# sungnyun/dualhyp

Hardware: AMD Instinct MI355X
Metric: corrected utterances/sec (TinyLlama-1.1B, 5+5 hyps, 512->64 tok) (higher is better)
Workload: dtype bf16; 1 GPU; DualHyp inference, TinyLlama-1.1B bf16 + LoRA r16 (q,k,v,proj), batch 32/GPU synthetic 5+5-hyp prompts, 512-token prompt -> 64 generated tokens, greedy; batch_per_gpu=32, parallelism=replicas x1, batches_in_flight_per_gpu=64, schedule=merged, decode_rows_per_launch=2048

## Files before the change

dualhyp_amd/_lib.py:

```python
from __future__ import annotations

import ctypes as C
from pathlib import Path

_HERE = Path(__file__).resolve().parent
import os as _os
LIB_PATH = Path(_os.environ["DUALHYP_HIP_LIB"]) if _os.environ.get("DUALHYP_HIP_LIB") else _HERE / "lib" / "libdualhyp_hip.so"

P = C.c_void_p
I = C.c_int
I64 = C.c_int64
U64 = C.c_uint64
F = C.c_float


class LayerWeights(C.Structure):
    _fields_ = [(n, P) for n in ("norm_1", "norm_2", "attn_w", "attn_lora_a", "attn_lora_b", "proj_w",
                                 "proj_lora_a", "proj_lora_b", "fc_1", "fc_2", "mlp_proj",
                                 "attn_ws", "proj_ws", "fc_1_ws", "fc_2_ws", "mlp_proj_ws")]


class ModelDesc(C.Structure):
    _fields_ = [("n_layer", C.c_int32), ("n_head", C.c_int32), ("n_groups", C.c_int32), ("head_size", C.c_int32),
                ("n_embd", C.c_int32), ("intermediate", C.c_int32), ("vocab", C.c_int32), ("block_size", C.c_int32),
# ... 24 lines not shown
    "dh_set_tuning": (I, [I, I]),
    "dh_debug_gemm_routes": (U64, [I]),
    "dh_last_error": (C.c_char_p, []),
    "dh_device_info": (I, [C.c_char_p, I, C.POINTER(I), C.POINTER(I64)]),
    "dh_embed_bf16": (I, [P, P, P, I, I, I, P]),
    "dh_rmsnorm_bf16": (I, [P, P, P, P, P, I, I, F, P, P]),
    "dh_qkv_rope_cache_bf16": (I, [P, P, P, P, P, P, P, P, P, P, I, I, I, I, I, P]),
    "dh_linear_bf16": (I, [P, P, P, I, I, I, I, P, P, I, P, F, I, I, P, P, P, P]),
    "dh_linear_qkv_rope_cache_bf16": (I, [P, P, I, I, P, I, P, F, P, P, P, P, P, P, P, I, I, I, I, P]),
    "dh_linear_lora_bf16": (I, [P, P, P, I, I, I, P, P, F, I, I, P, P, P]),
    "dh_linear_qkv_lora_rope_cache_bf16": (I, [P, P, I, I, P, P, F, P, P, P, P, P, P, P, I, I, I, I, P, P]),
    "dh_linear_partial_bf16": (I, [P, P, P, P, I, I, I, I, I, P]),
    "dh_linear_chain_bf16": (I, [P, P, P, P, I, I, I, I, I, P]),
    "dh_linear_partial_pairs_bf16": (I, [P, P, P, P, I, I, I, I, I, P]),
    "dh_finish_norm_bf16": (I, [P, I, I, I, I, I, P, F, P, P, P, P, F, P, P]),
    "dh_attn_decode_fused_bf16": (I, [P, I, I, I, I, I, P, F, I, I, P, P, P, P, P, P, P, I, I, I, I, P]),
    "dh_attn_verify_fused_bf16": (I, [P, I, I, I, I, I, I, P, F, I, I, P, P, P, P, P, P, P, I, I, I, I, I, P]),
    "dh_attn_prefill_bf16": (I, [P, P, P, P, P, P, P, P, P, I, I, I, I, I, I, P]),
    "dh_dropout_bf16": (I, [P, P, P, I64, F, C.c_uint64, C.c_uint32, P, P]),
    "dh_swiglu_fwd_bf16": (I, [P, P, P, I64, P]),
    "dh_linear_swiglu_train_bf16": (I, [P, P, P, P, P, P, I, I, I, P]),
    "dh_linear_mul_bf16": (I, [P, P, P, I, I, I, P, P]),
    "dh_swiglu_bwd_bf16": (I, [P, P, P, P, I, I, P]),
    "dh_rmsnorm_bwd_bf16": (I, [P, P, P, P, P, I, I, F, P]),
    "dh_qkv_rope_bwd_bf16": (I, [P, P, P, P, P, P, P, I, I, I, I, P]),
    "dh_tn_accum_f32": (I, [P, I, P, I, P, I, I, I, I, F, I, P, P]),
    "dh_tn_accum_work_bytes": (I64, [I, I, I]),
    "dh_tn_accum_seg_f32": (I, [P, I, P, I, P, I, I, I, I, I, F, I, P, P]),
    "dh_rowdot_f32": (I, [P, P, P, I64, I, P]),
    "dh_transpose_pad_bf16": (I, [P, P, P, P, P, I, I, I, I, P]),
# ... 115 lines not shown
```

dualhyp_amd/csrc/capi.hip:

```cpp
#include "common.h"
#include "tuning.h"
#include <stdarg.h>

static thread_local char g_err[512] = "";

void dh_set_error(const char* fmt, ...) {
    va_list ap;
    va_start(ap, fmt);
    vsnprintf(g_err, sizeof(g_err), fmt, ap);
    va_end(ap);
}

extern "C" const char* dh_last_error(void) { return g_err; }
extern "C" int dh_abi_version(void) { return DH_ABI_VERSION; }

int dh_stop_pack(const char* name, const dh_stop_spec* stop, bool start_ok, dh_stop_args& out) {
    out = dh_stop_args{};
    if (!stop) return 0;
    DH_CHECK(stop->n_seqs >= 0 && stop->n_seqs <= DH_MAX_STOP_SEQS, "%s: %d stop sequences, at most %d are supported", name, stop->n_seqs,
             DH_MAX_STOP_SEQS);
    DH_CHECK(stop->n_seqs == 0 || (stop->seqs && stop->h_seq_len), "%s: %d stop sequences without their ids or their lengths", name,
             stop->n_seqs);
    uint32_t lens = 0;
    for (int i = 0; i < stop->n_seqs; ++i) {
// ... 108 lines not shown
    {22, &g_w4_persist, RANGE, 0, 2, 0},
    {23, &g_prune_last_layer, BOOL, 0, 0, 0},
    {24, &g_w4_fast_epi, ANY, 0, 0, 0},
    {25, &g_w4_persist_qkv, BOOL, 0, 0, 0},
    {26, &g_tn_mfma, BOOL, 0, 0, 0},
    {27, &g_attn_bwd_dq_group, BOOL, 0, 0, 0},
    {28, &g_tail_split, BOOL, 0, 0, 0},
    {29, &g_attn_bwd_dkdv_img, BOOL, 0, 0, 0},
    {30, &g_w4_persist_lora, BOOL, 0, 0, 0},
    {31, &g_skinny_n, BOOL, 0, 0, 0},
    {40, &g_attn_chain, BOOL, 0, 0, 0},
    {41, &g_finish_hoist_rows, RANGE, -1, NO_MAX, 0},
    {42, &g_prefill_wpb, ONE_OF, 0, 2, 4},
    {43, &g_finish_rows_min, RANGE, -1, NO_MAX, 0},
    {44, &g_finish_rpb, RANGE, 0, 64, 0},
};

}

extern "C" int dh_set_tuning(int key, int value) {
    for (const TuningRow& r : TUNING) {
        if (r.key != key) continue;
        if (r.accept == RANGE && (value < r.a || value > r.b)) break;
        if (r.accept == ONE_OF && value != r.a && value != r.b && value != r.c) break;
        *r.knob = r.accept == BOOL ? value != 0 : value;
        return 0;
    }
    dh_set_error("dh_set_tuning: unknown key %d", key);
    return 1;
}
// ... 1 lines not shown
```

dualhyp_amd/csrc/decode_fused.hip:

```cpp
#include "common.h"
#include "tuning.h"

int g_attn_chain = 1;
int g_finish_hoist_rows = -1;
int g_finish_rows_min = -1;
int g_finish_rpb = 0;

#ifdef DH_ATTN_STAMPS
__device__ unsigned long long g_attn_stamps[4096 * 8];
#define ATTN_STAMP(i) do { if (threadIdx.x == 0 && blockIdx.x < 4096) g_attn_stamps[blockIdx.x * 8 + (i)] = __builtin_amdgcn_s_memrealtime(); } while (0)
#define ATTN_DRAIN() __builtin_amdgcn_s_waitcnt(0)
extern "C" int dh_debug_attn_stamps(unsigned long long* out) {
    return hipMemcpyFromSymbol(out, HIP_SYMBOL(g_attn_stamps), sizeof(g_attn_stamps)) == hipSuccess ? 0 : 1;
}
#else
#define ATTN_STAMP(i)
#define ATTN_DRAIN()
#endif

namespace {

constexpr int DCOLS = 16;
constexpr int MAXP = 16;

// ... 999 lines not shown
            const int c0 = (tid + i * 256) * 8;
            if (c0 < d) {
                const uint4 wu = i == 0 ? hwu : *reinterpret_cast<const uint4*>(w_norm + c0);
                const bf16_t* wp = reinterpret_cast<const bf16_t*>(&wu);
                uint4 o;
                bf16_t* op = reinterpret_cast<bf16_t*>(&o);
#pragma unroll
                for (int e = 0; e < 8; ++e) op[e] = f2bf(bf2f(wp[e]) * rbf(v[i][e] * r));
                *reinterpret_cast<uint4*>(xn_out + (size_t)row * d + c0) = o;
            }
        }
    };
    for (int k = 0; k < nrow; k += 2) {
        do_row(pa, pb, k);
        if (k + 1 < nrow) do_row(pb, pa, k + 1);
    }
}

}

extern "C" int dh_attn_decode_fused_bf16(const float* qkv32, int n_part, int pairs, int n_seq, int qkv_dim, int n_ext,
                                         const dh_bf16* lora_b, float lora_scale, int split0, int split1,
                                         const dh_bf16* cos, const dh_bf16* sin, const int32_t* seq_slot,
                                         const int32_t* kv_len, dh_bf16* k_cache, dh_bf16* vT_cache, dh_bf16* y,
                                         int n_head, int n_groups, int hs, int s_max, void* stream) {
    DH_CHECK(qkv32 && cos && sin && seq_slot && kv_len && k_cache && vT_cache && y, "dh_attn_decode_fused_bf16: null argument");
    DH_CHECK(n_groups > 0 && n_head % n_groups == 0 && n_head / n_groups <= DCOLS, "dh_attn_decode_fused_bf16: bad head counts");
    DH_CHECK(hs == 64 || hs == 96 || hs == 128, "dh_attn_decode_fused_bf16: head_size %d unsupported", hs);
    DH_CHECK(s_max % 64 == 0 && n_part >= 1 && n_part <= MAXP, "dh_attn_decode_fused_bf16: bad s_max / n_part");
    DH_CHECK(qkv_dim == (n_head + 2 * n_groups) * hs, "dh_attn_decode_fused_bf16: qkv_dim mismatch");
// ... 137 lines not shown
        else LAUNCH_MAXC(4);
#undef LAUNCH_MAXC
#undef LAUNCH_ROWS
        DH_LAUNCH_CHECK();
        return 0;
    }
    const int hoist_rows = g_finish_hoist_rows >= 0 ? g_finish_hoist_rows : FINISH_HOIST_ROWS;
    const bool hoist = hoist_rows > 0 && rows >= hoist_rows;
    if (d <= 2048) { LAUNCH(1); }
    else if (d <= 4096) { LAUNCH(2); }
    else { LAUNCH(4); }
#undef LAUNCH
    DH_LAUNCH_CHECK();
    return 0;
}
```

dualhyp_amd/csrc/engine.hip:

```cpp
#include <algorithm>
#include <mutex>
#include <vector>

#include "common.h"
#include "gemm.h"

constexpr int MAX_DECODE_ROWS = 2048;
int g_decode_tiled_rows = 0;
int g_short_kps = 8;
int g_fuse_qkv_rope = 1;
int g_prune_last_layer = 1;

struct dh_engine {
    dh_model_desc d;
    std::vector<dh_layer_weights> layers;
    int max_batch = 0, s_max = 0, max_tokens = 0;
    int row_cap = 0;
    int qkv_dim = 0, kv_dim = 0;
    bf16_t *kc = nullptr, *vtc = nullptr;
    bool kv8 = false;
    uint8_t *k8 = nullptr, *v8 = nullptr;
    int8_t *ke = nullptr, *ve = nullptr;
    size_t exp_layer_elems = 0;
    bf16_t *x = nullptr, *xn = nullptr, *qkv = nullptr, *qrot = nullptr, *att = nullptr, *xa = nullptr,
// ... 41 lines not shown
    hipStream_t gstream = nullptr;
    hipEvent_t ev_in = nullptr, ev_out = nullptr, ev_stage = nullptr;
    struct GKey {
        int64_t* tokens; int tok_ld; int32_t *length, *done; int n_seq, top_k; float temp; int64_t eos; uint64_t seed; int rsqrt_vec, tiled_rows;
        const int32_t *limit, *row_seq, *row_slot; int n_all, max_new;
        int spec; const int64_t* drafts; int32_t* counters;
        float* logprobs;
        int top_n; int32_t* top_ids; float* top_lp;
        const uint32_t* mask; int mask_ld;
        int ngram; const int32_t* ngram_start;
        dh_stop_args stop; const int32_t* stop_start; int32_t* stop_fin_tok;
        dh_nucleus_args nuc;
        dh_penalty_args pen; const int32_t* pen_start;
        dh_bias_args bias; const int32_t* bias_start;
        int beam_w; dh_beam_state beam;
        bool operator==(const GKey& k) const {
            return tokens == k.tokens && tok_ld == k.tok_ld && length == k.length && done == k.done && n_seq == k.n_seq &&
                   top_k == k.top_k && temp == k.temp && eos == k.eos && seed == k.seed && rsqrt_vec == k.rsqrt_vec &&
                   tiled_rows == k.tiled_rows && limit == k.limit && row_seq == k.row_seq && row_slot == k.row_slot &&
                   n_all == k.n_all && max_new == k.max_new && spec == k.spec && drafts == k.drafts && counters == k.counters &&
                   logprobs == k.logprobs && top_n == k.top_n && top_ids == k.top_ids && top_lp == k.top_lp && mask == k.mask &&
                   mask_ld == k.mask_ld && ngram == k.ngram && ngram_start == k.ngram_start && stop == k.stop && stop_start == k.stop_start &&
                   stop_fin_tok == k.stop_fin_tok && nuc == k.nuc && dh_penalty_same(pen, k.pen) && pen_start == k.pen_start &&
                   bias == k.bias && bias_start == k.bias_start &&
                   beam_w == k.beam_w &&
                   memcmp(&beam, &k.beam, sizeof(beam)) == 0;
        }
    };
    struct GEntry { GKey key; hipGraphExec_t exec; uint64_t used; };
    std::vector<GEntry> graphs;
    uint64_t graph_clock = 0;
    const int32_t* seq_slot = nullptr;
    bool capturing = false;
    bool phase_decode = false;
    bool decode_tiled = false;
    struct Timing {
        bool on = false;
        std::vector<std::pair<hipEvent_t, hipEvent_t>> ev[4];
    } tm;
};
// ... 467 lines not shown
            np = ks; pairs = 1;
            return dh_linear_partial_bf16(xin, w, wext, e->part32, n_seq, N, ext, K, ks, s);
        };
        int np, pairs;
        const int ext1 = W.attn_lora_a ? 48 : 0;
        if ((rc = partial(e->xn, W.attn_w, W.attn_lora_a, e->qkv_dim, ext1, d, pick_ksplit(d / 32), np, pairs))) return rc;
        if (spec_S > 1) {
            const int p_max = e->s_max < D.block_size ? e->s_max : D.block_size;
            if ((rc = dh_attn_verify_fused_impl(e->part32, np, pairs, n_seq / spec_S, spec_S, e->qkv_dim, ext1, W.attn_lora_b, D.lora_scale,
                                                d, d + e->kv_dim, D.rope_cos, D.rope_sin, m.seq_slot, m.kv, kc, vtc, e->att, H, G, hs,
                                                e->s_max, p_max, s))) return rc;
        } else
        if ((rc = dh_attn_decode_fused_bf16(e->part32, np, pairs, n_seq, e->qkv_dim, ext1, W.attn_lora_b, D.lora_scale, d,
                                            d + e->kv_dim, D.rope_cos, D.rope_sin, m.seq_slot, m.kv, kc, vtc, e->att, H, G,
                                            hs, e->s_max, s))) return rc;
        const int ext2 = W.proj_lora_a ? 16 : 0;
        if ((rc = partial(e->att, W.proj_w, W.proj_lora_a, d, ext2, d, pick_ksplit(d / 32), np, pairs))) return rc;
        if ((rc = dh_finish_norm_bf16(e->part32, np, pairs, n_seq, d, ext2, W.proj_lora_b, D.lora_scale, e->x, W.norm_2, e->x,
                                      e->xn, D.norm_eps, rt, s))) return rc;
        if ((rc = swiglu(e, e->xn, W.fc_1, W.fc_2, e->act, n_seq, I, d, s, false))) return rc;
        if ((rc = partial(e->act, W.mlp_proj, nullptr, d, 0, I, pick_ksplit(I / 32), np, pairs))) return rc;
        const bf16_t* next_norm = l + 1 < D.n_layer ? e->layers[l + 1].norm_1 : D.ln_f;
        if ((rc = dh_finish_norm_bf16(e->part32, np, pairs, n_seq, d, 0, nullptr, 0.f, e->x, next_norm, e->x, e->xn,
                                      D.norm_eps, rt, s))) return rc;
    }
    return 0;
}

int head(dh_engine* e, const bf16_t* xrows, int rows, bf16_t* logits, const uint8_t* tail_flags, hipStream_t s) {
    const dh_model_desc& D = e->d;
    const uint8_t* rt = e->rsqrt_vec > 0 ? tail_flags : nullptr;
    int rc;
    if (e->fp8) {
        if ((rc = dh_rmsnorm_quant_fp8(xrows, D.ln_f, e->xn, e->xq, e->xscale, rows, D.n_embd, D.norm_eps, rt, s))) return rc;
        TimeScope t(e, gemm_class(e), s);
        return dh_linear_fp8_ex(e->xq, e->xscale, reinterpret_cast<const uint8_t*>(D.lm_head), D.lm_head_ws, logits, rows, D.vocab,
                                D.n_embd, DH_EPI_ADAPTER, nullptr, nullptr, D.adapter_scale, D.adapter_bias, nullptr,
                                fp8_kernel(e->phase_decode, rows), s);
    }
// ... 796 lines not shown
```

dualhyp_amd/csrc/gemm.h:

```cpp
#pragma once
#include "common.h"
#include "tuning.h"

struct GemmArgs {
    const bf16_t* x;
    const bf16_t* w;
    const bf16_t* w2;
    bf16_t* y;
    const bf16_t* xa;
    const bf16_t* lora_a;
    const bf16_t* lora_b;
    const bf16_t* vec_a;
    const bf16_t* vec_b;
    const bf16_t* resid;
    int M, N, K;
    int xa_ld, split0, split1;
    float lora_scale;
    int nb_n, nb_m;
    int gm;
    int fast_epi;
    int resid_mul;
    const bf16_t* rope_cos;
    const bf16_t* rope_sin;
    const int32_t* tok_slot;
// ... 41 lines not shown
bool dh_linear_k64_ok(int M, int N, int K, const void* x, const void* w, const void* y, const void* mul);
int dh_linear_k64(const dh_bf16* x, const dh_bf16* w, const dh_bf16* mul, dh_bf16* y, int M, int N, hipStream_t s);
bool dh_linear_256_xa_ok(const GemmArgs& a, int epilogue);

bool dh_linear_mid_ok(const GemmArgs& a, int epilogue);
int dh_linear_mid(const GemmArgs& a, int epilogue, hipStream_t s);

bool dh_linear_dt_ok(const GemmArgs& a, int epilogue, int seg);
int dh_linear_dt(const GemmArgs& a, int epilogue, int seg, hipStream_t s);
bool dh_chain_ok(int M, int n_main, int n_ext, int K, int ksplit);
bool dh_pairs_ok(int M, int n_main, int n_ext, int K, int ksplit);
int dh_pairs_tiled(const bf16_t* x, const bf16_t* w, const bf16_t* w_ext, float* y32, int M, int n_main, int n_ext, int K,
                   int kps, hipStream_t s);
int dh_chain_tiled(const bf16_t* x, const bf16_t* w, const bf16_t* w_ext, float* y32, int M, int n_main, int n_ext, int K,
                   int kps, hipStream_t s);

bool dh_linear_is_big(int M, int N, int epilogue);

int dh_linear_256(GemmArgs a, int epilogue, hipStream_t s);

int dh_linear_lora_impl(const dh_bf16* x, const dh_bf16* w, dh_bf16* y, int M, int N, int K, const dh_bf16* lora_a, const dh_bf16* lora_b,
                        float lora_scale, int split0, int split1, const dh_bf16* resid, dh_bf16* xa_work, int kernel, hipStream_t s);
int dh_linear_impl(const dh_bf16* x, const dh_bf16* w, dh_bf16* y, int M, int N, int K, int epilogue,
                   const dh_bf16* w2, const dh_bf16* xa, int xa_ld, const dh_bf16* lora_b, float lora_scale,
                   int split0, int split1, const dh_bf16* vec_a, const dh_bf16* vec_b, const dh_bf16* resid,
                   int kernel, hipStream_t s);
```

dualhyp_amd/csrc/gemm_dt.hip:

```cpp
#include "common.h"
#include "gemm.h"

int g_dt_stages = 0;
int g_dt_wide = 0;

namespace {

constexpr int TB = 128;
constexpr int BKD = 64;
template <int WN> constexpr int stage_bytes() { return (WN * 64 + TB) * BKD * 2; }

__device__ __forceinline__ int swz7(int row) { return (row >> 1) & 7; }

struct DtArgs {
    const bf16_t* x;
    const bf16_t* w;
    const bf16_t* w2;
    void* y;
    const bf16_t* vec_a;
    const bf16_t* vec_b;
    const bf16_t* resid;
    int M, N, K, n_main, seg;
    int split_kt;
    int wt;
};

template <int MODE, int NSTAGE, int WN, int WI>
__device__ __forceinline__ void gemm_dt_body(const DtArgs& a) {
    static_assert(WI == 4 || (WI == 2 && MODE == 0 && !(WN == 4 && NSTAGE == 3)), "the 32 x 64 wave tile serves MODE 0 on the plain ring");
    constexpr int STAGE = stage_bytes<WN>();
    constexpr int ASZ = WN * 64 * BKD * 2;
    constexpr int NWV = WN * 8 / WI;
    constexpr int NA = WI;
    constexpr int NB = 16 / NWV;
    constexpr int PER = NA + NB;
    extern __shared__ __attribute__((aligned(16))) char smem[];
    const int tid = threadIdx.x, lane = tid & 63;
    const int wave = WI == 2 ? __builtin_amdgcn_readfirstlane(tid >> 6) : tid >> 6;
    const int wn = wave >> 1, wm = wave & 1;
    const int frow = lane & 15, kg = lane >> 4;
    const int m_tiles = (a.M + TB - 1) / TB;
    int tile, ky = 0;
    {
        const int nwg = gridDim.x * gridDim.y, bid = blockIdx.x + gridDim.x * blockIdx.y, xcd = bid & 7, q = nwg >> 3, r = nwg & 7;
        tile = (xcd < r ? xcd * (q + 1) : r * (q + 1) + (xcd - r) * q) + (bid >> 3);
        if (MODE == 4) { ky = tile / (int)gridDim.x; tile -= ky * (int)gridDim.x; }
    }
    const int tm = tile % m_tiles, tn = tile / m_tiles;
    const int m0 = tm * TB;
    const int n0 = MODE == 1 ? tn * (WN * 32) : tn * (WN * 64);
// ... 16 lines not shown
            n = n0 + row;
            n = n < a.N ? n : a.N - 1;
            if ((MODE == 0 || MODE == 4) && n >= a.n_main) { base = a.w2; n -= a.n_main; }
        }
        srcA[j] = base + (size_t)n * a.K + chunk * 8 + (MODE == 4 ? (size_t)ky * a.split_kt * BKD : 0);
    }
#pragma unroll
    for (int j = 0; j < NB; ++j) {
        const int R = wave * NB + j;
        const int row = R * 8 + (lane >> 3);
        const int chunk = (lane & 7) ^ swz7(row);
        int m = m0 + row;
        m = m < a.M ? m : a.M - 1;
        srcB[j] = a.x + (size_t)m * a.K + chunk * 8 + (MODE == 4 ? (size_t)ky * a.split_kt * BKD : 0);
    }
    auto stage = [&](int kt) __attribute__((always_inline)) {
        char* sA = smem + (kt % NSTAGE) * STAGE;
        char* sB = sA + ASZ;
#pragma unroll
        for (int j = 0; j < NA; ++j) glds16(srcA[j] + kt * BKD, sA + (wave * NA + j) * 1024);
#pragma unroll
        for (int j = 0; j < NB; ++j) glds16(srcB[j] + kt * BKD, sB + (wave * NB + j) * 1024);
    };
    auto wait_next = [&](int ahead) __attribute__((always_inline)) {
        if (NSTAGE >= 4 && ahead >= 2) asm volatile("s_waitcnt vmcnt(%0)" ::"n"(2 * PER) : "memory");
        else if (NSTAGE >= 3 && ahead >= 1) asm volatile("s_waitcnt vmcnt(%0)" ::"n"(PER) : "memory");
        else asm volatile("s_waitcnt vmcnt(0)" ::: "memory");
    };

    f32x4 cur[WI][4], tot[WI][4];
#pragma unroll
    for (int i = 0; i < WI; ++i)
#pragma unroll
        for (int j = 0; j < 4; ++j) {
            cur[i][j] = f32x4{0.f, 0.f, 0.f, 0.f};
            tot[i][j] = f32x4{0.f, 0.f, 0.f, 0.f};
        }
    const int sw = swz7(frow);
    const int offA = (wn * (WI * 16) + frow) * 128, offB = (wm * 64 + frow) * 128;
    const int nk = MODE == 4 ? min(a.split_kt, a.K / BKD - ky * a.split_kt) : a.K / BKD;
    const int seg_kt = a.seg / 2;
    f32x4 pairacc[MODE == 0 ? WI : 1][MODE == 0 ? 4 : 1];
    int seg_idx = 0;

    auto fold_segment = [&](bool last) __attribute__((always_inline)) {
        if (MODE == 0) {
            const bool second = seg_idx & 1;
#pragma unroll
            for (int i = 0; i < WI; ++i)
#pragma unroll
                for (int j = 0; j < 4; ++j) {
                    if (second) tot[i][j] += pairacc[i][j] + cur[i][j];
                    else if (last) tot[i][j] += cur[i][j];
                    else pairacc[i][j] = cur[i][j];
                    cur[i][j] = f32x4{0.f, 0.f, 0.f, 0.f};
                }
            ++seg_idx;
        } else {
#pragma unroll
            for (int i = 0; i < WI; ++i)
#pragma unroll
                for (int j = 0; j < 4; ++j) {
                    tot[i][j] += cur[i][j];
                    cur[i][j] = f32x4{0.f, 0.f, 0.f, 0.f};
                }
        }
    };
    int in_seg = 0;
    if constexpr (WN == 4 && NSTAGE == 3) {
    auto stage_w = [&](int kt) __attribute__((always_inline)) {
        char* sA = smem + (kt % NSTAGE) * STAGE;
// ... 52 lines not shown
        if (p < nk) stage(p);
    wait_next((nk < NSTAGE - 1 ? nk : NSTAGE - 1) - 1);
    __builtin_amdgcn_s_barrier();
    for (int kt = 0; kt < nk; ++kt) {
        const bool pre = kt + NSTAGE - 1 < nk;
        const char* sA = smem + (kt % NSTAGE) * STAGE;
        const char* sB = sA + ASZ;
        if (pre) stage(kt + NSTAGE - 1);
#pragma unroll
        for (int ks = 0; ks < 2; ++ks) {
            const int co = ((ks * 4 + kg) ^ sw) << 4;
            if constexpr (WI == 2) {
                bf16x8 fa[2];
#pragma unroll
                for (int i = 0; i < 2; ++i) fa[i] = *reinterpret_cast<const bf16x8*>(sA + offA + i * 2048 + co);
#pragma unroll
                for (int j = 0; j < 4; ++j) {
                    const bf16x8 fb = *reinterpret_cast<const bf16x8*>(sB + offB + j * 2048 + co);
#pragma unroll
                    for (int i = 0; i < 2; ++i) cur[i][j] = __builtin_amdgcn_mfma_f32_16x16x32_bf16(fa[i], fb, cur[i][j], 0, 0, 0);
                }
            } else {
            bf16x8 fa[4], fb[4];
#pragma unroll
            for (int i = 0; i < 4; ++i) {
                fa[i] = *reinterpret_cast<const bf16x8*>(sA + offA + i * 2048 + co);
                fb[i] = *reinterpret_cast<const bf16x8*>(sB + offB + i * 2048 + co);
            }
#pragma unroll
            for (int i = 0; i < 4; ++i)
// ... 2 lines not shown
                    cur[i][j] = __builtin_amdgcn_mfma_f32_16x16x32_bf16(fa[i], fb[j], cur[i][j], 0, 0, 0);
            }
        }
        if (++in_seg == seg_kt || kt + 1 == nk) {
            in_seg = 0;
            fold_segment(kt + 1 == nk);
        }
        {
            const int issued = (kt + NSTAGE - 1 < nk ? kt + NSTAGE - 1 : nk - 1);
            wait_next(issued - (kt + 1));
        }
        __builtin_amdgcn_s_barrier();
    }
    }

#pragma unroll
    for (int j = 0; j < 4; ++j) {
        const int m = m0 + wm * 64 + j * 16 + frow;
        if (m >= a.M) continue;
        if constexpr (MODE == 1) {
#pragma unroll
            for (int i = 0; i < 2; ++i) {
                const int n = n0 + wn * 32 + i * 16 + kg * 4;
                if (n >= a.N) continue;
                float o[4];
#pragma unroll
                for (int r = 0; r < 4; ++r) {
                    const float gt = rbf(tot[i][j][r]), up = rbf(tot[i + 2][j][r]);
                    o[r] = rbf(silu_fast(gt)) * up;
                }
// ... 23 lines not shown
#pragma unroll
                    for (int r = 0; r < 4; ++r) o[r] = bf2f(rp[r]) + o[r];
                }
                *reinterpret_cast<uint2*>((bf16_t*)a.y + (size_t)m * a.N + n) = make_uint2(pack2bf(o[0], o[1]), pack2bf(o[2], o[3]));
            }
        }
    }
}

template <int MODE, int NSTAGE, int WN = 2>
__global__ __launch_bounds__(WN * 128) void gemm_dt_kernel(DtArgs a) { gemm_dt_body<MODE, NSTAGE, WN, 4>(a); }

template <int NSTAGE>
__global__ __launch_bounds__(512, NSTAGE == 2 ? 4 : 2) void gemm_dt_chain_kernel(DtArgs a) { gemm_dt_body<0, NSTAGE, 2, 2>(a); }

template <int NSTAGE>
int launch_chain_n(const DtArgs& a, int blocks, hipStream_t s) {
    constexpr int lds = NSTAGE * stage_bytes<2>();
    DH_MAX_LDS_ONCE((gemm_dt_chain_kernel<NSTAGE>), lds);
    dh_gemm_route(DH_ROUTE_CHAIN_TILED);
    hipLaunchKernelGGL((gemm_dt_chain_kernel<NSTAGE>), dim3(blocks), dim3(512), lds, s, a);
    DH_LAUNCH_CHECK();
    return 0;
}

template <int MODE, int NSTAGE, int WN = 2>
int launch_dt_n(const DtArgs& a, int blocks, hipStream_t s, int ny = 1) {
    constexpr int lds = NSTAGE * stage_bytes<WN>();
    DH_MAX_LDS_ONCE((gemm_dt_kernel<MODE, NSTAGE, WN>), lds);
    dh_gemm_route(MODE == 0 ? DH_ROUTE_CHAIN_TILED : MODE == 4 ? DH_ROUTE_PAIRS_TILED : DH_ROUTE_DT_FUSED);
// ... 12 lines not shown
    const int stages = g_dt_stages ? g_dt_stages : (blocks > 256 ? 2 : 4);
    return stages == 2 ? launch_dt_n<MODE, 2>(a, blocks, s) : launch_dt_n<MODE, 4>(a, blocks, s);
}

}

int g_dt_min_rows = 129;
int g_chain_min_rows = 1536;

int dh_chain_tiled(const bf16_t* x, const bf16_t* w, const bf16_t* w_ext, float* y32, int M, int n_main, int n_ext, int K,
                   int kps, hipStream_t s) {
    DtArgs a{x, w, w_ext ? w_ext : w, y32, nullptr, nullptr, nullptr, M, n_main + n_ext, K, n_main, kps, 0, 0};
    const int blocks = cdiv(M, TB) * cdiv(a.N, TB);
    const int stages = g_dt_stages ? g_dt_stages : (blocks > 256 ? 2 : 4);
    return stages == 2 ? launch_chain_n<2>(a, blocks, s) : launch_chain_n<4>(a, blocks, s);
}

int g_pairs_wn = 0;
int g_pairs_wt = 0;
int dh_pairs_tiled(const bf16_t* x, const bf16_t* w, const bf16_t* w_ext, float* y32, int M, int n_main, int n_ext, int K,
                   int kps, hipStream_t s) {
    const int N = n_main + n_ext, nslices = cdiv(K / 32, kps), ny = (nslices + 1) / 2;
    DtArgs a{x, w, w_ext ? w_ext : w, y32, nullptr, nullptr, nullptr, M, N, K, n_main, kps, kps, g_pairs_wt};
    const int m_tiles = cdiv(M, TB);
    const int wide_blocks = m_tiles * cdiv(N, 256) * ny;
    const bool wide = g_pairs_wn ? g_pairs_wn == 4 : wide_blocks >= 160;
    if (wide) return launch_dt_n<4, 3, 4>(a, m_tiles * cdiv(N, 256), s, ny);
    const int blocks = m_tiles * cdiv(N, TB);
    return blocks * ny > 256 ? launch_dt_n<4, 2>(a, blocks, s, ny) : launch_dt_n<4, 4>(a, blocks, s, ny);
}
// ... 17 lines not shown
```

dualhyp_amd/csrc/gemm_skinny.hip:

```cpp
#include "common.h"
#include "gemm.h"

int g_skinny_variant = 1;
int g_swiglu2 = 1;
int g_rows_ng = 0;
int g_rows_ct = 0;

namespace {

constexpr int ROWS = 16;
constexpr int NW = 8;
constexpr int CH = 8;

template <int EPI, bool RESID>
__global__ __launch_bounds__(512, 2) void gemm_skinny_kernel(GemmArgs a) {
    __shared__ __attribute__((aligned(16))) float part[NW][32][ROWS];
    __shared__ __attribute__((aligned(16))) float part2[EPI == DH_EPI_SWIGLU ? NW : 1][32][ROWS];
    const int tid = threadIdx.x, lane = tid & 63, wave = tid >> 6;
    const int n0 = blockIdx.x * ROWS;
    const int lrow = lane & 15, kg = lane >> 4;
    constexpr bool SW = EPI == DH_EPI_SWIGLU;
    constexpr int CHK = SW ? CH / 2 : CH;
    const int kw = wave, kstride = NW;
    int n = n0 + lrow;
// ... 571 lines not shown
             n_ext % ROWS == 0, "dh_linear_partial_pairs_bf16: unsupported shape N=%d+%d K=%d ksplit=%d (K %% 64 == 0, whole K-slices of 8 or 16 k-steps)",
             n_main, n_ext, K, ksplit);
    return dh_pairs_tiled(x, w, w_ext, y32, M, n_main, n_ext, K, kps, (hipStream_t)stream);
}

extern "C" int dh_linear_chain_bf16(const dh_bf16* x, const dh_bf16* w, const dh_bf16* w_ext, float* y32, int M, int n_main,
                                    int n_ext, int K, int ksplit, void* stream) {
    DH_CHECK(x && w && y32 && M >= 1 && ksplit >= 1 && (n_ext == 0 || w_ext), "dh_linear_chain_bf16: bad argument");
    DH_CHECK(dh_chain_ok(M, n_main, n_ext, K, ksplit),
             "dh_linear_chain_bf16: unsupported shape M=%d N=%d+%d K=%d ksplit=%d (needs >= %d rows, K %% 64 == 0, K-slices of 8 or 16 k-steps)",
             M, n_main, n_ext, K, ksplit, g_chain_min_rows);
    const int kps = (K / 32 + ksplit - 1) / ksplit;
    return dh_chain_tiled(x, w, w_ext, y32, M, n_main, n_ext, K, kps, (hipStream_t)stream);
}

int g_skinny_n = 1;
bool dh_linear_skinny_n_ok(int M, int N, int K, const void* x, const void* w, const void* y) {
    return g_skinny_n && N >= 16 && N <= 64 && N % 16 == 0 && M >= 512 && K >= 64 && K % 64 == 0 && (size_t)M * K * 2 < (1ull << 32) &&
           (((uintptr_t)x | (uintptr_t)w) & 15) == 0 && ((uintptr_t)y & 7) == 0;
}
int dh_linear_skinny_n(const dh_bf16* x, const dh_bf16* w, dh_bf16* y, int M, int N, int K, hipStream_t s) {
    const dim3 grid(cdiv(M, 64)), block(256);
    const int nt = N / 16, lds = 4 * (64 * 128 + nt * 16 * 128);
    dh_gemm_route(DH_ROUTE_SKINNY_N);
    switch (nt) {
        case 1: hipLaunchKernelGGL((gemm_skinny_n_kernel<1>), grid, block, lds, s, x, w, y, M, K, N); break;
        case 2: hipLaunchKernelGGL((gemm_skinny_n_kernel<2>), grid, block, lds, s, x, w, y, M, K, N); break;
        case 3: hipLaunchKernelGGL((gemm_skinny_n_kernel<3>), grid, block, lds, s, x, w, y, M, K, N); break;
        default: hipLaunchKernelGGL((gemm_skinny_n_kernel<4>), grid, block, lds, s, x, w, y, M, K, N); break;
    }
// ... 35 lines not shown
```

dualhyp_amd/csrc/tuning.h:

```cpp
#pragma once

extern int g_gemm128_stages, g_gemm_variant, g_tail_split, g_linear_phase;
extern int g_gemm_gm, g_w4_persist, g_w4_fast_epi, g_w4_persist_qkv, g_w4_persist_lora;
extern int g_mid, g_mid_wlds;
extern int g_dt_stages, g_dt_wide, g_dt_min_rows, g_chain_min_rows, g_pairs_wn, g_pairs_wt;
extern int g_pairs_min_rows, g_skinny_n;
__attribute__((visibility("hidden"))) extern int g_skinny_variant, g_swiglu2, g_rows_ct, g_rows_ng;
extern int g_fp8_tile, g_fp8_gm;
extern int g_decode_tiled_rows, g_short_kps, g_fuse_qkv_rope, g_prune_last_layer;
extern int g_attn_bwd_dkdv_img, g_attn_bwd_dq_group;
extern int g_tn_mfma;
extern int g_attn_chain, g_finish_hoist_rows, g_finish_rows_min, g_finish_rpb;
extern int g_prefill_wpb;
```

dualhyp_amd/ops.py:

```python
from __future__ import annotations

import os
from typing import Sequence, Optional, Tuple

import torch

from . import _lib
from ._lib import check

EPI_PLAIN, EPI_LORA, EPI_SWIGLU, EPI_ADAPTER = 0, 1, 2, 3


def _p(t: Optional[torch.Tensor]):
    return None if t is None else t.data_ptr()


def _stream() -> int:
    return torch.cuda.current_stream().cuda_stream


def _dev(t: torch.Tensor, dtype=torch.bfloat16, name="tensor") -> torch.Tensor:
    if not t.is_cuda:
        raise _lib.DualHypHipError(f"{name} must live on the GPU: the HIP path has no CPU fallback")
    if t.dtype != dtype:
# ... 692 lines not shown
    return y


def finish_norm(h32: torch.Tensor, d: int, x_resid: torch.Tensor, w_norm: torch.Tensor, eps: float,
                lora_b: Optional[torch.Tensor] = None, lora_scale: float = 1.0,
                row_tail: Optional[torch.Tensor] = None, pairs: bool = True) -> Tuple[torch.Tensor, torch.Tensor]:
    k = _Keep()
    n_part, rows, ld = h32.shape
    x_resid = _dev(x_resid, name="x_resid")
    x_out, xn_out = torch.empty_like(x_resid), torch.empty_like(x_resid)
    check(_lib.load().dh_finish_norm_bf16(_p(h32), n_part, int(pairs), rows, d, ld - d, _p(lora_b), float(lora_scale), _p(x_resid),
                                          k(w_norm), _p(x_out), _p(xn_out), float(eps), _p(row_tail), _stream()))
    return x_out, xn_out


def attn_decode_fused(qkv32: torch.Tensor, qkv_dim: int, lora_b: Optional[torch.Tensor], lora_scale: float,
                      splits: Tuple[int, int], cos: torch.Tensor, sin: torch.Tensor, seq_slot: torch.Tensor,
                      kv_len: torch.Tensor, k_cache: torch.Tensor, vT_cache: torch.Tensor, n_head: int,
                      pairs: bool = True) -> torch.Tensor:
    k = _Keep()
    n_part, n_seq, ld = qkv32.shape
    n_groups, s_max, hs = k_cache.size(1), k_cache.size(2), k_cache.size(3)
    y = torch.empty((n_seq, n_head * hs), dtype=torch.bfloat16, device=qkv32.device)
    i32 = torch.int32
    check(_lib.load().dh_attn_decode_fused_bf16(_p(qkv32), n_part, int(pairs), n_seq, qkv_dim, ld - qkv_dim, _p(lora_b),
                                                float(lora_scale), splits[0], splits[1], k(cos), k(sin),
                                                k(seq_slot, i32), k(kv_len, i32), _p(k_cache), _p(vT_cache),
                                                _p(y), n_head, n_groups, hs, s_max, _stream()))
    return y

# ... 156 lines not shown
```

include/dualhyp_hip.h:

```cpp
#ifndef DUALHYP_HIP_H
#define DUALHYP_HIP_H

#include <stdint.h>

#ifdef __cplusplus
extern "C" {
#endif

typedef uint16_t dh_bf16;

#define DH_ABI_VERSION 6

int dh_abi_version(void);
int dh_set_tuning(int key, int value);
uint64_t dh_debug_gemm_routes(int reset);
const char* dh_last_error(void);
int dh_device_info(char* h_buf, int h_buf_len, int* h_num_cu, int64_t* h_hbm_bytes);


int dh_embed_bf16(const int64_t* ids, const dh_bf16* wte, dh_bf16* out, int n_tok, int d,
                  int vocab, void* stream);

int dh_rmsnorm_bf16(const dh_bf16* x, const dh_bf16* resid, const dh_bf16* w, dh_bf16* out,
                    dh_bf16* sum_out, int rows, int d, float eps, const uint8_t* row_tail,
// ... 29 lines not shown
                                       const int32_t* tok_slot, const int32_t* tok_pos, dh_bf16* q_out, dh_bf16* k_cache,
                                       dh_bf16* vT_cache, int n_head, int n_groups, int hs, int s_max, dh_bf16* xa_work,
                                       void* stream);

int dh_linear_partial_bf16(const dh_bf16* x, const dh_bf16* w, const dh_bf16* w_ext, float* y32,
                           int M, int n_main, int n_ext, int K, int ksplit, void* stream);
int dh_linear_partial_pairs_bf16(const dh_bf16* x, const dh_bf16* w, const dh_bf16* w_ext, float* y32, int M,
                                 int n_main, int n_ext, int K, int ksplit, void* stream);
int dh_linear_chain_bf16(const dh_bf16* x, const dh_bf16* w, const dh_bf16* w_ext, float* y32, int M,
                         int n_main, int n_ext, int K, int ksplit, void* stream);

int dh_finish_norm_bf16(const float* h32, int n_part, int pairs, int rows, int d, int n_ext,
                        const dh_bf16* lora_b, float lora_scale, const dh_bf16* x_resid,
                        const dh_bf16* w_norm, dh_bf16* x_out, dh_bf16* xn_out, float eps,
                        const uint8_t* row_tail, void* stream);


int dh_attn_prefill_bf16(const dh_bf16* q, const dh_bf16* k_cache, const dh_bf16* vT_cache,
                         const int32_t* seq_slot, const int32_t* q_start, const int32_t* q_len,
                         const int32_t* kv_pos0, dh_bf16* y, float* lse, int n_seq, int max_q_len,
                         int n_head, int n_groups, int hs, int s_max, void* stream);

int64_t dh_attn_decode_work_bytes(int n_seq, int n_head, int hs, int s_max);
int dh_attn_decode_bf16(const dh_bf16* q, const dh_bf16* k_cache, const dh_bf16* vT_cache,
                        const int32_t* seq_slot, const int32_t* kv_len, dh_bf16* y, void* work,
                        int n_seq, int n_head, int n_groups, int hs, int s_max, void* stream);

int dh_attn_decode_fused_bf16(const float* qkv32, int n_part, int pairs, int n_seq, int qkv_dim, int n_ext,
                              const dh_bf16* lora_b, float lora_scale, int split0, int split1,
                              const dh_bf16* cos, const dh_bf16* sin, const int32_t* seq_slot,
// ... 347 lines not shown
```

Before: 855.5 utterances/s.

## Fuse residual add and LoRA epilogue into chain GEMM, then separate RMSNorm

In decode, the out-projection and MLP down-projection no longer write fp32 partial sums and reduce them in a finish-norm kernel when the chain shape allows it. A new finishing mode of the tiled chain GEMM computes the LoRA x·A product alongside the main MFMA loop and adds LoRA B plus the residual in its epilogue, writing bf16 x in place. A lightweight row-wise RMSNorm kernel then produces xn. This removes the fp32 partial-buffer traffic, at the cost of an extra norm launch and a heavier GEMM epilogue that adds LDS and register pressure.

```diff
diff --git a/dualhyp_amd/_lib.py b/dualhyp_amd/_lib.py
--- a/dualhyp_amd/_lib.py
+++ b/dualhyp_amd/_lib.py
@@ -62,6 +62,8 @@
     "dh_linear_chain_bf16": (I, [P, P, P, P, I, I, I, I, I, P]),
     "dh_linear_partial_pairs_bf16": (I, [P, P, P, P, I, I, I, I, I, P]),
     "dh_finish_norm_bf16": (I, [P, I, I, I, I, I, P, F, P, P, P, P, F, P, P]),
+    "dh_linear_chain_finish_bf16": (I, [P, P, P, P, F, P, I, I, I, I, P]),
+    "dh_norm_finished_bf16": (I, [P, P, P, I, I, F, P, P]),
     "dh_attn_decode_fused_bf16": (I, [P, I, I, I, I, I, P, F, I, I, P, P, P, P, P, P, P, I, I, I, I, P]),
     "dh_attn_verify_fused_bf16": (I, [P, I, I, I, I, I, I, P, F, I, I, P, P, P, P, P, P, P, I, I, I, I, I, P]),
     "dh_attn_prefill_bf16": (I, [P, P, P, P, P, P, P, P, P, I, I, I, I, I, I, P]),
diff --git a/dualhyp_amd/csrc/capi.hip b/dualhyp_amd/csrc/capi.hip
--- a/dualhyp_amd/csrc/capi.hip
+++ b/dualhyp_amd/csrc/capi.hip
@@ -146,6 +146,7 @@
     {42, &g_prefill_wpb, ONE_OF, 0, 2, 4},
     {43, &g_finish_rows_min, RANGE, -1, NO_MAX, 0},
     {44, &g_finish_rpb, RANGE, 0, 64, 0},
+    {45, &g_chain_finish, BOOL, 0, 0, 0},
 };
 
 }
diff --git a/dualhyp_amd/csrc/decode_fused.hip b/dualhyp_amd/csrc/decode_fused.hip
--- a/dualhyp_amd/csrc/decode_fused.hip
+++ b/dualhyp_amd/csrc/decode_fused.hip
@@ -1037,6 +1037,70 @@
     for (int k = 0; k < nrow; k += 2) {
         do_row(pa, pb, k);
         if (k + 1 < nrow) do_row(pb, pa, k + 1);
+    }
+}
+
+template <int MAXC>
+__global__ __launch_bounds__(256) void norm_finished_rows_kernel(const bf16_t* __restrict__ x, const bf16_t* __restrict__ w_norm,
+                                                                 bf16_t* __restrict__ xn_out, int rows, int d, float eps,
+                                                                 const uint8_t* __restrict__ row_tail, int rpb) {
+    __shared__ float sRed[2][4];
+    const int tid = threadIdx.x, lane = tid & 63, wave = tid >> 6;
+    const int row0 = blockIdx.x * rpb, nrow = min(rpb, rows - row0);
+    uint4 wu[MAXC], xc[MAXC], xq[MAXC];
+#pragma unroll
+    for (int i = 0; i < MAXC; ++i) {
+        const int c0 = (tid + i * 256) * 8;
+        wu[i] = xc[i] = xq[i] = make_uint4(0u, 0u, 0u, 0u);
+        if (c0 < d) {
+            xc[i] = *reinterpret_cast<const uint4*>(x + (size_t)row0 * d + c0);
+            wu[i] = *reinterpret_cast<const uint4*>(w_norm + c0);
+        }
+    }
+    for (int k = 0; k < nrow; ++k) {
+        const int row = row0 + k, par = k & 1;
+        if (k + 1 < nrow) {
+#pragma unroll
+            for (int i = 0; i < MAXC; ++i) {
+                const int c0 = (tid + i * 256) * 8;
+                if (c0 < d) xq[i] = *reinterpret_cast<const uint4*>(x + (size_t)(row + 1) * d + c0);
+            }
+        }
+        const bool tail = row_tail != nullptr && row_tail[row] != 0;
+        float v[MAXC][8];
+        float ss = 0.f;
+#pragma unroll
+        for (int i = 0; i < MAXC; ++i) {
+            const int c0 = (tid + i * 256) * 8;
+            if (c0 < d) {
+                const bf16_t* xp = reinterpret_cast<const bf16_t*>(&xc[i]);
+#pragma unroll
+                for (int e = 0; e < 8; ++e) {
+                    v[i][e] = bf2f(xp[e]);
+                    ss += rbf(v[i][e] * v[i][e]);
+                }
+            }
+        }
+        ss = wave_sum(ss);
+        if (lane == 0) sRed[par][wave] = ss;
+        __syncthreads();
+        ss = sRed[par][0] + sRed[par][1] + sRed[par][2] + sRed[par][3];
+        const float ms = rbf(ss / (float)d);
+        const float t = rbf(ms + eps);
+        const float r = tail ? rbf(1.0f / rbf(sqrtf(t))) : rbf(1.0f / sqrtf(t));
+#pragma unroll
+        for (int i = 0; i < MAXC; ++i) {
+            const int c0 = (tid + i * 256) * 8;
+            if (c0 < d) {
+                const bf16_t* wp = reinterpret_cast<const bf16_t*>(&wu[i]);
+                uint4 o;
+                bf16_t* op = reinterpret_cast<bf16_t*>(&o);
+#pragma unroll
+                for (int e = 0; e < 8; ++e) op[e] = f2bf(bf2f(wp[e]) * rbf(v[i][e] * r));
+                *reinterpret_cast<uint4*>(xn_out + (size_t)row * d + c0) = o;
+            }
+            xc[i] = xq[i];
+        }
     }
 }
 
@@ -1204,3 +1268,19 @@
     DH_LAUNCH_CHECK();
     return 0;
 }
+
+extern "C" int dh_norm_finished_bf16(const dh_bf16* x, const dh_bf16* w_norm, dh_bf16* xn_out, int rows, int d, float eps,
+                                     const uint8_t* row_tail, void* stream) {
+    DH_CHECK(x && w_norm && xn_out, "dh_norm_finished_bf16: null argument");
+    DH_CHECK(d % 8 == 0 && d > 0 && d <= 8192, "dh_norm_finished_bf16: unsupported d=%d", d);
+    if (rows <= 0) return 0;
+    hipStream_t s = (hipStream_t)stream;
+    const int multi_rows = g_finish_rows_min >= 0 ? g_finish_rows_min : FINISH_ROWS_MIN;
+    const int rpb = multi_rows > 0 && rows >= multi_rows ? (g_finish_rpb > 0 ? g_finish_rpb : FINISH_RPB) : 1;
+    const dim3 grid((rows + rpb - 1) / rpb), block(256);
+    if (d <= 2048) hipLaunchKernelGGL((norm_finished_rows_kernel<1>), grid, block, 0, s, x, w_norm, xn_out, rows, d, eps, row_tail, rpb);
+    else if (d <= 4096) hipLaunchKernelGGL((norm_finished_rows_kernel<2>), grid, block, 0, s, x, w_norm, xn_out, rows, d, eps, row_tail, rpb);
+    else hipLaunchKernelGGL((norm_finished_rows_kernel<4>), grid, block, 0, s, x, w_norm, xn_out, rows, d, eps, row_tail, rpb);
+    DH_LAUNCH_CHECK();
+    return 0;
+}
diff --git a/dualhyp_amd/csrc/engine.hip b/dualhyp_amd/csrc/engine.hip
--- a/dualhyp_amd/csrc/engine.hip
+++ b/dualhyp_amd/csrc/engine.hip
@@ -79,6 +79,7 @@
         dh_penalty_args pen; const int32_t* pen_start;
         dh_bias_args bias; const int32_t* bias_start;
         int beam_w; dh_beam_state beam;
+        int chain_finish = g_chain_finish;
         bool operator==(const GKey& k) const {
             return tokens == k.tokens && tok_ld == k.tok_ld && length == k.length && done == k.done && n_seq == k.n_seq &&
                    top_k == k.top_k && temp == k.temp && eos == k.eos && seed == k.seed && rsqrt_vec == k.rsqrt_vec &&
@@ -88,7 +89,7 @@
                    mask_ld == k.mask_ld && ngram == k.ngram && ngram_start == k.ngram_start && stop == k.stop && stop_start == k.stop_start &&
                    stop_fin_tok == k.stop_fin_tok && nuc == k.nuc && dh_penalty_same(pen, k.pen) && pen_start == k.pen_start &&
                    bias == k.bias && bias_start == k.bias_start &&
-                   beam_w == k.beam_w &&
+                   beam_w == k.beam_w && chain_finish == k.chain_finish &&
                    memcmp(&beam, &k.beam, sizeof(beam)) == 0;
         }
     };
@@ -586,15 +587,21 @@
         if ((rc = dh_attn_decode_fused_bf16(e->part32, np, pairs, n_seq, e->qkv_dim, ext1, W.attn_lora_b, D.lora_scale, d,
                                             d + e->kv_dim, D.rope_cos, D.rope_sin, m.seq_slot, m.kv, kc, vtc, e->att, H, G,
                                             hs, e->s_max, s))) return rc;
-        const int ext2 = W.proj_lora_a ? 16 : 0;
-        if ((rc = partial(e->att, W.proj_w, W.proj_lora_a, d, ext2, d, pick_ksplit(d / 32), np, pairs))) return rc;
-        if ((rc = dh_finish_norm_bf16(e->part32, np, pairs, n_seq, d, ext2, W.proj_lora_b, D.lora_scale, e->x, W.norm_2, e->x,
-                                      e->xn, D.norm_eps, rt, s))) return rc;
+        auto linear_finish_norm = [&](const bf16_t* xin, const bf16_t* w, const bf16_t* la, const bf16_t* lb, int K, const bf16_t* w_norm) {
+            const int ext = la ? 16 : 0, ks = pick_ksplit(K / 32);
+            int r;
+            if (g_chain_finish && dh_chain_ok(n_seq, d, ext, K, ks)) {
+                if ((r = dh_linear_chain_finish_bf16(xin, w, la, la ? lb : nullptr, D.lora_scale, e->x, n_seq, d, K, ks, s))) return r;
+                return dh_norm_finished_bf16(e->x, w_norm, e->xn, n_seq, d, D.norm_eps, rt, s);
+            }
+            if ((r = partial(xin, w, la, d, ext, K, ks, np, pairs))) return r;
+            return dh_finish_norm_bf16(e->part32, np, pairs, n_seq, d, ext, la ? lb : nullptr, la ? D.lora_scale : 0.f, e->x, w_norm, e->x,
+                                       e->xn, D.norm_eps, rt, s);
+        };
+        if ((rc = linear_finish_norm(e->att, W.proj_w, W.proj_lora_a, W.proj_lora_b, d, W.norm_2))) return rc;
         if ((rc = swiglu(e, e->xn, W.fc_1, W.fc_2, e->act, n_seq, I, d, s, false))) return rc;
-        if ((rc = partial(e->act, W.mlp_proj, nullptr, d, 0, I, pick_ksplit(I / 32), np, pairs))) return rc;
         const bf16_t* next_norm = l + 1 < D.n_layer ? e->layers[l + 1].norm_1 : D.ln_f;
-        if ((rc = dh_finish_norm_bf16(e->part32, np, pairs, n_seq, d, 0, nullptr, 0.f, e->x, next_norm, e->x, e->xn,
-                                      D.norm_eps, rt, s))) return rc;
+        if ((rc = linear_finish_norm(e->act, W.mlp_proj, nullptr, nullptr, I, next_norm))) return rc;
     }
     return 0;
 }
diff --git a/dualhyp_amd/csrc/gemm.h b/dualhyp_amd/csrc/gemm.h
--- a/dualhyp_amd/csrc/gemm.h
+++ b/dualhyp_amd/csrc/gemm.h
@@ -79,6 +79,8 @@
                    int kps, hipStream_t s);
 int dh_chain_tiled(const bf16_t* x, const bf16_t* w, const bf16_t* w_ext, float* y32, int M, int n_main, int n_ext, int K,
                    int kps, hipStream_t s);
+int dh_chain_finish_tiled(const bf16_t* x, const bf16_t* w, const bf16_t* lora_a, const bf16_t* lora_b, float lora_scale, bf16_t* x_io,
+                          int M, int N, int K, int kps, hipStream_t s);
 
 bool dh_linear_is_big(int M, int N, int epilogue);
 
diff --git a/dualhyp_amd/csrc/gemm_dt.hip b/dualhyp_amd/csrc/gemm_dt.hip
--- a/dualhyp_amd/csrc/gemm_dt.hip
+++ b/dualhyp_amd/csrc/gemm_dt.hip
@@ -23,17 +23,21 @@
     int M, N, K, n_main, seg;
     int split_kt;
     int wt;
+    float lora_scale;
 };
 
 template <int MODE, int NSTAGE, int WN, int WI>
 __device__ __forceinline__ void gemm_dt_body(const DtArgs& a) {
-    static_assert(WI == 4 || (WI == 2 && MODE == 0 && !(WN == 4 && NSTAGE == 3)), "the 32 x 64 wave tile serves MODE 0 on the plain ring");
-    constexpr int STAGE = stage_bytes<WN>();
+    constexpr bool FIN = MODE == 5 || MODE == 6;
+    constexpr bool XA = MODE == 6, CHAIN = MODE == 0 || FIN;
+    static_assert(WI == 4 || (WI == 2 && CHAIN && !(WN == 4 && NSTAGE == 3)), "the 32 x 64 wave tile serves the chain modes on the plain ring");
+    static_assert(!FIN || (WI == 2 && WN == 2), "the finishing modes run on the register-lean tile");
+    constexpr int STAGE = stage_bytes<WN>() + (XA ? 16 * BKD * 2 : 0);
     constexpr int ASZ = WN * 64 * BKD * 2;
     constexpr int NWV = WN * 8 / WI;
     constexpr int NA = WI;
     constexpr int NB = 16 / NWV;
-    constexpr int PER = NA + NB;
+    constexpr int PER = NA + NB + (XA ? 1 : 0);
     extern __shared__ __attribute__((aligned(16))) char smem[];
     const int tid = threadIdx.x, lane = tid & 63;
     const int wave = WI == 2 ? __builtin_amdgcn_readfirstlane(tid >> 6) : tid >> 6;
@@ -80,6 +84,11 @@
         m = m < a.M ? m : a.M - 1;
         srcB[j] = a.x + (size_t)m * a.K + chunk * 8 + (MODE == 4 ? (size_t)ky * a.split_kt * BKD : 0);
     }
+    const bf16_t* srcL = nullptr;
+    if constexpr (XA) {
+        const int row = wave * 2 + (lane >> 5), p = lane & 31;
+        srcL = a.w2 + (size_t)row * a.K + (((p >> 2) ^ swz7(row)) * 8 + (p & 3) * 2);
+    }
     auto stage = [&](int kt) __attribute__((always_inline)) {
         char* sA = smem + (kt % NSTAGE) * STAGE;
         char* sB = sA + ASZ;
@@ -87,6 +96,9 @@
         for (int j = 0; j < NA; ++j) glds16(srcA[j] + kt * BKD, sA + (wave * NA + j) * 1024);
 #pragma unroll
         for (int j = 0; j < NB; ++j) glds16(srcB[j] + kt * BKD, sB + (wave * NB + j) * 1024);
+        if constexpr (XA)
+            __builtin_amdgcn_global_load_lds((const __attribute__((address_space(1))) void*)(srcL + kt * BKD),
+                                             (__attribute__((address_space(3))) void*)(sB + TB * BKD * 2 + wave * 256), 4, 0, 0);
     };
     auto wait_next = [&](int ahead) __attribute__((always_inline)) {
         if (NSTAGE >= 4 && ahead >= 2) asm volatile("s_waitcnt vmcnt(%0)" ::"n"(2 * PER) : "memory");
@@ -106,11 +118,13 @@
     const int offA = (wn * (WI * 16) + frow) * 128, offB = (wm * 64 + frow) * 128;
     const int nk = MODE == 4 ? min(a.split_kt, a.K / BKD - ky * a.split_kt) : a.K / BKD;
     const int seg_kt = a.seg / 2;
-    f32x4 pairacc[MODE == 0 ? WI : 1][MODE == 0 ? 4 : 1];
+    f32x4 pairacc[CHAIN ? WI : 1][CHAIN ? 4 : 1];
+    f32x4 xcur = {0.f, 0.f, 0.f, 0.f}, xpair = {0.f, 0.f, 0.f, 0.f}, xtot = {0.f, 0.f, 0.f, 0.f};
+    const int offX = (wm * 64 + wn * 16 + frow) * 128;
     int seg_idx = 0;
 
     auto fold_segment = [&](bool last) __attribute__((always_inline)) {
-        if (MODE == 0) {
+        if (CHAIN) {
             const bool second = seg_idx & 1;
 #pragma unroll
             for (int i = 0; i < WI; ++i)
@@ -121,6 +135,12 @@
                     else pairacc[i][j] = cur[i][j];
                     cur[i][j] = f32x4{0.f, 0.f, 0.f, 0.f};
                 }
+            if constexpr (XA) {
+                if (second) xtot += xpair + xcur;
+                else if (last) xtot += xcur;
+                else xpair = xcur;
+                xcur = f32x4{0.f, 0.f, 0.f, 0.f};
+            }
             ++seg_idx;
         } else {
 #pragma unroll
@@ -203,6 +223,11 @@
                 bf16x8 fa[2];
 #pragma unroll
                 for (int i = 0; i < 2; ++i) fa[i] = *reinterpret_cast<const bf16x8*>(sA + offA + i * 2048 + co);
+                if constexpr (XA) {
+                    const bf16x8 fx = *reinterpret_cast<const bf16x8*>(sB + TB * BKD * 2 + frow * 128 + co);
+                    const bf16x8 fbx = *reinterpret_cast<const bf16x8*>(sB + offX + co);
+                    xcur = __builtin_amdgcn_mfma_f32_16x16x32_bf16(fx, fbx, xcur, 0, 0, 0);
+                }
 #pragma unroll
                 for (int j = 0; j < 4; ++j) {
                     const bf16x8 fb = *reinterpret_cast<const bf16x8*>(sB + offB + j * 2048 + co);
@@ -235,6 +260,66 @@
     }
     }
 
+    if constexpr (FIN) {
+        float* sX = reinterpret_cast<float*>(smem);
+        if constexpr (XA) {
+            f32x4 v;
+#pragma unroll
+            for (int r = 0; r < 4; ++r) v[r] = rbf(0.f + xtot[r]);
+            *reinterpret_cast<f32x4*>(sX + (wm * 64 + wn * 16 + frow) * 16 + kg * 4) = v;
+            __syncthreads();
+        }
+        bf16_t* xio = (bf16_t*)a.y;
+#pragma unroll
+        for (int i = 0; i < WI; ++i) {
+            const int n = n0 + wn * (WI * 16) + i * 16 + kg * 4;
+            if (n >= a.N) continue;
+            uint4 bq[XA ? 4 : 1][2];
+            if constexpr (XA) {
+#pragma unroll
+                for (int r = 0; r < 4; ++r) {
+                    const uint4* b4 = reinterpret_cast<const uint4*>(a.vec_a + (size_t)(n + r) * 16);
+                    bq[r][0] = b4[0];
+                    bq[r][1] = b4[1];
+                }
+            }
+#pragma unroll
+            for (int j = 0; j < 4; ++j) {
+                const int ml = wm * 64 + j * 16 + frow, m = m0 + ml;
+                if (m >= a.M) continue;
+                const uint2 rv = *reinterpret_cast<const uint2*>(a.resid + (size_t)m * a.N + n);
+                const bf16_t* rp = reinterpret_cast<const bf16_t*>(&rv);
+                float xa[XA ? 16 : 1];
+                if constexpr (XA) {
+#pragma unroll
+                    for (int q = 0; q < 4; ++q) {
+                        const f32x4 v = *reinterpret_cast<const f32x4*>(sX + ml * 16 + q * 4);
+#pragma unroll
+                        for (int r = 0; r < 4; ++r) xa[q * 4 + r] = v[r];
+                    }
+                }
+                float o[4];
+#pragma unroll
+                for (int r = 0; r < 4; ++r) {
+                    o[r] = rbf(0.f + tot[i][j][r]);
+                    if constexpr (XA) {
+                        float l = 0.f;
+#pragma unroll
+                        for (int h = 0; h < 2; ++h) {
+                            const uint4 bv = bq[r][h];
+                            const bf16_t* bp = reinterpret_cast<const bf16_t*>(&bv);
+#pragma unroll
+                            for (int k = 0; k < 8; ++k) l = fmaf(xa[h * 8 + k], bf2f(bp[k]), l);
+                        }
+                        o[r] = rbf(o[r] + rbf(rbf(l) * a.lora_scale));
+                    }
+                    o[r] = bf2f(rp[r]) + o[r];
+                }
+                *reinterpret_cast<uint2*>(xio + (size_t)m * a.N + n) = make_uint2(pack2bf(o[0], o[1]), pack2bf(o[2], o[3]));
+            }
+        }
+        return;
+    }
 #pragma unroll
     for (int j = 0; j < 4; ++j) {
         const int m = m0 + wm * 64 + j * 16 + frow;
@@ -288,6 +373,19 @@
 template <int NSTAGE>
 __global__ __launch_bounds__(512, NSTAGE == 2 ? 4 : 2) void gemm_dt_chain_kernel(DtArgs a) { gemm_dt_body<0, NSTAGE, 2, 2>(a); }
 
+template <bool LORA>
+__global__ __launch_bounds__(512, 2) void gemm_dt_finish_kernel(DtArgs a) { gemm_dt_body<LORA ? 6 : 5, 4, 2, 2>(a); }
+
+template <bool LORA>
+int launch_finish(const DtArgs& a, int blocks, hipStream_t s) {
+    constexpr int lds = 4 * (stage_bytes<2>() + (LORA ? 16 * BKD * 2 : 0));
+    DH_MAX_LDS_ONCE((gemm_dt_finish_kernel<LORA>), lds);
+    dh_gemm_route(DH_ROUTE_CHAIN_TILED);
+    hipLaunchKernelGGL((gemm_dt_finish_kernel<LORA>), dim3(blocks), dim3(512), lds, s, a);
+    DH_LAUNCH_CHECK();
+    return 0;
+}
+
 template <int NSTAGE>
 int launch_chain_n(const DtArgs& a, int blocks, hipStream_t s) {
     constexpr int lds = NSTAGE * stage_bytes<2>();
@@ -330,6 +428,14 @@
     const int blocks = cdiv(M, TB) * cdiv(a.N, TB);
     const int stages = g_dt_stages ? g_dt_stages : (blocks > 256 ? 2 : 4);
     return stages == 2 ? launch_chain_n<2>(a, blocks, s) : launch_chain_n<4>(a, blocks, s);
+}
+
+int g_chain_finish = 1;
+int dh_chain_finish_tiled(const bf16_t* x, const bf16_t* w, const bf16_t* lora_a, const bf16_t* lora_b, float lora_scale, bf16_t* x_io,
+                          int M, int N, int K, int kps, hipStream_t s) {
+    DtArgs a{x, w, lora_a ? lora_a : w, x_io, lora_b, nullptr, x_io, M, N, K, N, kps, 0, 0, lora_scale};
+    const int blocks = cdiv(M, TB) * cdiv(N, TB);
+    return lora_a ? launch_finish<true>(a, blocks, s) : launch_finish<false>(a, blocks, s);
 }
 
 int g_pairs_wn = 0;
diff --git a/dualhyp_amd/csrc/gemm_skinny.hip b/dualhyp_amd/csrc/gemm_skinny.hip
--- a/dualhyp_amd/csrc/gemm_skinny.hip
+++ b/dualhyp_amd/csrc/gemm_skinny.hip
@@ -609,6 +609,16 @@
     return dh_chain_tiled(x, w, w_ext, y32, M, n_main, n_ext, K, kps, (hipStream_t)stream);
 }
 
+extern "C" int dh_linear_chain_finish_bf16(const dh_bf16* x, const dh_bf16* w, const dh_bf16* lora_a, const dh_bf16* lora_b,
+                                           float lora_scale, dh_bf16* x_io, int M, int N, int K, int ksplit, void* stream) {
+    DH_CHECK(x && w && x_io && M >= 1 && ksplit >= 1 && (lora_a == nullptr) == (lora_b == nullptr), "dh_linear_chain_finish_bf16: bad argument");
+    DH_CHECK(dh_chain_ok(M, N, lora_a ? 16 : 0, K, ksplit),
+             "dh_linear_chain_finish_bf16: unsupported shape M=%d N=%d K=%d ksplit=%d (needs >= %d rows, K %% 64 == 0, K-slices of 8 or 16 k-steps)",
+             M, N, K, ksplit, g_chain_min_rows);
+    const int kps = (K / 32 + ksplit - 1) / ksplit;
+    return dh_chain_finish_tiled(x, w, lora_a, lora_b, lora_scale, x_io, M, N, K, kps, (hipStream_t)stream);
+}
+
 int g_skinny_n = 1;
 bool dh_linear_skinny_n_ok(int M, int N, int K, const void* x, const void* w, const void* y) {
     return g_skinny_n && N >= 16 && N <= 64 && N % 16 == 0 && M >= 512 && K >= 64 && K % 64 == 0 && (size_t)M * K * 2 < (1ull << 32) &&
diff --git a/dualhyp_amd/csrc/tuning.h b/dualhyp_amd/csrc/tuning.h
--- a/dualhyp_amd/csrc/tuning.h
+++ b/dualhyp_amd/csrc/tuning.h
@@ -3,7 +3,7 @@
 extern int g_gemm128_stages, g_gemm_variant, g_tail_split, g_linear_phase;
 extern int g_gemm_gm, g_w4_persist, g_w4_fast_epi, g_w4_persist_qkv, g_w4_persist_lora;
 extern int g_mid, g_mid_wlds;
-extern int g_dt_stages, g_dt_wide, g_dt_min_rows, g_chain_min_rows, g_pairs_wn, g_pairs_wt;
+extern int g_dt_stages, g_dt_wide, g_dt_min_rows, g_chain_min_rows, g_pairs_wn, g_pairs_wt, g_chain_finish;
 extern int g_pairs_min_rows, g_skinny_n;
 __attribute__((visibility("hidden"))) extern int g_skinny_variant, g_swiglu2, g_rows_ct, g_rows_ng;
 extern int g_fp8_tile, g_fp8_gm;
diff --git a/dualhyp_amd/ops.py b/dualhyp_amd/ops.py
--- a/dualhyp_amd/ops.py
+++ b/dualhyp_amd/ops.py
@@ -730,6 +730,26 @@
     return x_out, xn_out
 
 
+def linear_chain_finish(x: torch.Tensor, w: torch.Tensor, x_io: torch.Tensor, ksplit: int, lora_a: Optional[torch.Tensor] = None,
+                        lora_b: Optional[torch.Tensor] = None, lora_scale: float = 1.0) -> torch.Tensor:
+    x, w = _dev(x, name="x"), _dev(w, name="w")
+    K = x.size(-1)
+    M = x.numel() // K
+    assert x_io.is_contiguous() and x_io.dtype == torch.bfloat16 and tuple(x_io.shape) == (M, w.size(0))
+    check(_lib.load().dh_linear_chain_finish_bf16(_p(x), _p(w), _p(lora_a), _p(lora_b), float(lora_scale), _p(x_io), M, w.size(0), K,
+                                                  ksplit, _stream()))
+    return x_io
+
+
+def norm_finished(x: torch.Tensor, w_norm: torch.Tensor, eps: float, row_tail: Optional[torch.Tensor] = None) -> torch.Tensor:
+    k = _Keep()
+    x = _dev(x, name="x")
+    rows, d = x.shape
+    xn = torch.empty_like(x)
+    check(_lib.load().dh_norm_finished_bf16(_p(x), k(w_norm), _p(xn), rows, d, float(eps), _p(row_tail), _stream()))
+    return xn
+
+
 def attn_decode_fused(qkv32: torch.Tensor, qkv_dim: int, lora_b: Optional[torch.Tensor], lora_scale: float,
                       splits: Tuple[int, int], cos: torch.Tensor, sin: torch.Tensor, seq_slot: torch.Tensor,
                       kv_len: torch.Tensor, k_cache: torch.Tensor, vT_cache: torch.Tensor, n_head: int,
diff --git a/include/dualhyp_hip.h b/include/dualhyp_hip.h
--- a/include/dualhyp_hip.h
+++ b/include/dualhyp_hip.h
@@ -67,6 +67,11 @@
                         const dh_bf16* lora_b, float lora_scale, const dh_bf16* x_resid,
                         const dh_bf16* w_norm, dh_bf16* x_out, dh_bf16* xn_out, float eps,
                         const uint8_t* row_tail, void* stream);
+
+int dh_linear_chain_finish_bf16(const dh_bf16* x, const dh_bf16* w, const dh_bf16* lora_a, const dh_bf16* lora_b,
+                                float lora_scale, dh_bf16* x_io, int M, int N, int K, int ksplit, void* stream);
+int dh_norm_finished_bf16(const dh_bf16* x, const dh_bf16* w_norm, dh_bf16* xn_out, int rows, int d, float eps,
+                          const uint8_t* row_tail, void* stream);
 
 
 int dh_attn_prefill_bf16(const dh_bf16* q, const dh_bf16* k_cache, const dh_bf16* vT_cache,
```

Result: no change. 862.0 utterances/s, median of 6 (+0.8%).
